# bhmm/bhmm

Hardware: NVIDIA B200
Metric: Baum-Welch EM throughput (frames x iterations per second) (higher is better)
Workload: dtype f64

## Files before the change

bhmm_b200/csrc/engine.cu:

```cuda
#include <algorithm>
#include <cstdio>
#include <cstdlib>
#include <cstring>

#include "host_common.h"
#include "../../include/bhmm_b200.h"

struct bhmm_b200_batch {
    int K = 0, N = 0;
    long long rows = 0;
    std::vector<long long> offsets;
    int chunk = 0, warm_f = 0, warm_b = 0, warm_min = 32;
    int req_chunk = 0, req_warm = 0;
    int vit_phase = 0;
    bool vit_map_chunked = false;
    std::vector<int> vit_end;
    bool lane = false;
    bool no_alpha = false;
    double* d_g0buf = nullptr;
    int partial_rows = 0;
    HostPlan plan, segplan;
    Arena arena;
    bool carved = false;
    char* cw_base = nullptr;
// ... 65 lines not shown
        b->d_sigma = (double*)(base + o_sg);
        b->d_partials = (double*)(base + o_part);
        b->d_g0buf = (double*)(base + o_g0);
        b->d_err = (int*)(base + o_err);
        b->d_alpha = (double*)(base + o_alpha);
        b->d_F = (unsigned char*)(base + o_F);
        b->d_vflag = (unsigned*)(base + o_vflag);
        b->cw_base = base + o_cw;
    }
    return cv.off + 256;
}

int batch_carve(bhmm_b200_batch* b, cudaStream_t st)
{
    if (b->carved) return BHMM_OK;
    const size_t need = batch_layout(b, nullptr);
    RC_TRY(b->arena.ensure(need));
    batch_layout(b, b->arena.base);
    RC_TRY(chainwork_setup(b->w, b->plan, b->N, b->warm_f, b->cw_base, st));
    const int ns = b->segplan.n;
    CUDA_TRY(cudaMemcpyAsync(b->d_offsets, b->offsets.data(), sizeof(long long) * (b->K + 1), cudaMemcpyHostToDevice, st));
    CUDA_TRY(cudaMemcpyAsync((void*)b->seg.row0, b->segplan.row0.data(), sizeof(long long) * ns, cudaMemcpyHostToDevice, st));
    CUDA_TRY(cudaMemcpyAsync((void*)b->seg.len, b->segplan.len.data(), sizeof(int) * ns, cudaMemcpyHostToDevice, st));
    CUDA_TRY(cudaMemcpyAsync((void*)b->seg.t0, b->segplan.t0.data(), sizeof(int) * ns, cudaMemcpyHostToDevice, st));
    CUDA_TRY(cudaMemcpyAsync((void*)b->seg.T, b->segplan.T.data(), sizeof(int) * ns, cudaMemcpyHostToDevice, st));
    CUDA_TRY(cudaStreamSynchronize(st));
    b->carved = true;
    return BHMM_OK;
}

void batch_plan(bhmm_b200_batch* b, int chunk, int warm)
{
    b->req_chunk = chunk;
    b->req_warm = warm;
    const int w = warm > 0 ? warm : (b->lane ? auto_warm_lane(b->N) : auto_warm(b->N));
    b->chunk = chunk > 0 ? chunk : (b->lane ? auto_chunk_lane(b->rows, b->N, w) : auto_chunk(b->rows, b->N, w));
    if (chunk <= 0) {
        int sms = 148, dev = 0;
        if (cudaGetDevice(&dev) == cudaSuccess) cudaDeviceGetAttribute(&sms, cudaDevAttrMultiProcessorCount, dev);
        int tthreads = 32, tcpb = 1;
        team_shape(b->N, &tthreads, &tcpb);
        const long long cap = b->lane ? (long long)sms * lane_blocks_per_sm(b->N, EM_GAUSS) * lane_threads()
                                      : (long long)backward_stats_grid(b->N, 1 << 28) * tcpb;
        auto count = [&](long long c) {
            long long n = 0;
            for (int k = 0; k < b->K; ++k) {
                const long long own = b->own_lo.empty() ? b->offsets[k + 1] - b->offsets[k] : b->own_hi[k] - b->own_lo[k];
                n += (own + c - 1) / c;
            }
            return n;
        };
        if (b->lane) {
            for (int it = 0; it < 200; ++it) {
                if (count(b->chunk) <= cap || b->chunk >= (1 << 30)) break;
                b->chunk = (int)std::min<long long>((long long)b->chunk + std::max(1, b->chunk / 100), 1 << 30);
            }
        } else {
            long long maxT = 1;
            for (int k = 0; k < b->K; ++k) maxT = std::max(maxT, b->offsets[k + 1] - b->offsets[k]);
            const long long lo_c = std::max<long long>(64, 2LL * w);
            double best_cost = 1e300;
            long long best_c = std::max<long long>(maxT, 1);
            for (int m = 1; m <= 32; ++m) {
                if (count(maxT) > (long long)m * cap) continue;
                long long lo = std::min(lo_c, maxT), hi = maxT;
                while (lo < hi) {
                    const long long mid = (lo + hi) / 2;
                    if (count(mid) <= (long long)m * cap) hi = mid; else lo = mid + 1;
                }
                const double cost = (double)m * ((double)lo + (lo < maxT ? (double)w : 0.0));
                if (cost < best_cost * 0.98) { best_cost = cost; best_c = lo; }
            }
            b->chunk = (int)std::min<long long>(best_c, 1 << 30);
        }
    }
    b->warm_f = b->warm_b = w;
    b->warm_min = warm > 0 ? warm : 32;
    build_plan(b->offsets.data(), b->K, b->chunk, b->plan, b->own_lo.empty() ? nullptr : b->own_lo.data(),
               b->own_hi.empty() ? nullptr : b->own_hi.data());
    build_plan(b->offsets.data(), b->K, SEG_FRAMES, b->segplan);
    b->carved = false;
}

int upload_small(double* dst, const double* src, size_t n, cudaStream_t st)
{
    CUDA_TRY(cudaMemcpyAsync(dst, src, sizeof(double) * n, cudaMemcpyHostToDevice, st));
    return BHMM_OK;
}

struct ScanGuard {
    bhmm_b200_batch* b;
    ScanGuard(bhmm_b200_batch* b_, const Emission& em, int emkind) : b(b_)
    {
        const int N = b->N;
        static int off = -1;
        if (off < 0) { const char* e = getenv("BHMM_B200_EXACT_SCAN"); off = (e && e[0] == '0') ? 1 : 0; }
        if (off || !exact_scan_ok(N) || !b->w.chunked) return;
        b->w.scan = [this, &em, emkind, N](int dir, cudaStream_t st) -> int {
            const size_t need = exact_scan_bytes(b->w.n_total, N);
            if (b->scan.ensure(need) != BHMM_OK) { bhmm_set_error(BHMM_ERR_NO_MEM, "exact scan: device memory for the chain operators"); return BHMM_ERR_NO_MEM; }
            Chains all = b->w.ch;
            return launch_exact_scan(all, b->w.n_total, em, emkind, b->d_A, N, dir, dir > 0 ? b->w.he_f : b->w.he_b,
                                     reinterpret_cast<double*>(b->scan.base), st);
        };
    }
    ~ScanGuard() { b->w.scan = nullptr; }
};

struct RepairTolGuard {
    ChainWork& w;
    explicit RepairTolGuard(ChainWork& w_) : w(w_) { w.repair_tol = g_repair_tol; }
    ~RepairTolGuard() { w.repair_tol = 0.0; }
};

void begin_info(bhmm_b200_batch* b)
{
    b->info = RunInfo();
    b->info.chains = b->plan.n;
    b->info.chunk = b->chunk;
    b->info.warm = b->warm_f;
}

int prepare_discrete(bhmm_b200_batch* b, const double* B, int M, Emission& em, cudaStream_t st)
{
    const int N = b->N;
    RC_TRY(b->disc.ensure(sizeof(double) * 2 * (size_t)N * M + 512));
    double* stage = (double*)b->disc.base;
    double* Bt = stage + (((size_t)N * M + 31) & ~(size_t)31);
    CUDA_TRY(cudaMemcpyAsync(stage, B, sizeof(double) * (size_t)N * M, cudaMemcpyHostToDevice, st));
    RC_TRY(launch_transpose(stage, N, M, Bt, st));
    LAUNCHED(1);
    em.Bt = Bt;
    em.M = M;
    return BHMM_OK;
}

int estep_common(bhmm_b200_batch* b, Emission& em, int emkind, const double* A, const double* pi, const double* mu,
                 const double* sigma, double* d_gamma, double* d_stats, double* d_Bnum, cudaStream_t st)
{
    const int N = b->N;
    if (b->no_alpha) { bhmm_set_error(BHMM_ERR_UNSUPPORTED, "Viterbi-only batch: no forward variables"); return BHMM_ERR_UNSUPPORTED; }
    RC_TRY(upload_small(b->d_A, A, (size_t)N * N, st));
    RC_TRY(upload_small(b->d_pi, pi, N, st));
    b->w.ch.warm = b->warm_f;
    ScanGuard scan_guard(b, em, emkind);
    RepairTolGuard repair_guard(b->w);
    LaneArgs la{};
    LaneHostParams hp{A, pi, mu, sigma};
    if (b->lane) {
        la.obs = em.obs; la.sym = em.sym; la.Bt = em.Bt; la.M = em.M; la.ignore_outliers = em.ignore_outliers;
        la.alpha_il = b->d_alpha; la.Lmax = b->chunk; la.alpha_rm = nullptr;
        la.chain_ll = b->w.chain_ll; la.g0buf = b->d_g0buf; la.partials = b->d_partials;
        la.Bnum = d_Bnum; la.gamma = d_gamma;
    }
    static int optimistic = -1;
    if (optimistic < 0) { const char* e = getenv("BHMM_B200_OPTIMISTIC"); optimistic = (e && e[0] == '1') ? 1 : 0; }
    auto launch_fwd = [&](const Chains& ch, cudaStream_t s2) -> int {
        if (b->lane) {
            LaneArgs x = la;
            x.ch = ch; x.hand_used = b->w.hu_f; x.hand_end = b->w.he_f;
            return launch_lane(x, hp, N, emkind, LANE_FORWARD, s2);
        }
        FwdArgs a{};
        a.ch = ch; a.em = em; a.N = N; a.A = b->d_A; a.pi = b->d_pi; a.alpha = b->d_alpha;
        a.chain_ll = b->w.chain_ll; a.hand_used = b->w.hu_f; a.hand_end = b->w.he_f;
        return launch_forward_team(a, emkind, s2);
    };
    auto launch_bwd = [&](const Chains& ch, cudaStream_t s2) -> int {
        if (b->lane) {
            LaneArgs x = la;
            x.ch = ch; x.hand_used = b->w.hu_b; x.hand_end = b->w.he_b;
            return launch_lane(x, hp, N, emkind, LANE_BACKWARD_STATS, s2);
        }
        BwdArgs a{};
        a.ch = ch;
        a.em = em; a.N = N; a.grid = b->stats_grid; a.A = b->d_A;
        a.alpha = b->d_alpha; a.gamma = d_gamma; a.Bnum = d_Bnum; a.partials = b->d_partials;
        a.hand_used = b->w.hu_b; a.hand_end = b->w.he_b;
        return launch_backward_team(a, emkind, true, s2);
    };
    auto finalize = [&]() -> int {
        const int prow = b->lane ? lane_blocks(b->w.n_total) : b->stats_grid;
        RC_TRY(launch_finalize_stats(b->d_partials, prow, b->w.chain_ll, b->w.n_total, b->d_A, N, d_stats, st));
        LAUNCHED(1);
        if (b->lane) {
            RC_TRY(launch_add_gamma0(b->w.ch, b->w.n_total, N, b->d_g0buf, d_stats, st));
            LAUNCHED(1);
        }
        return BHMM_OK;
    };
    if (optimistic && b->w.chunked) {
        Chains all = b->w.ch;
        all.list = nullptr; all.n = b->w.n_total; all.exact = 0; all.warmv = nullptr;
        b->w.need_f = b->w.need_b = 0.0;
        if (b->profile) cudaEventRecord(b->ev[0], st);
        all.warm = b->warm_f;
        RC_TRY(launch_fwd(all, st));
        LAUNCHED(1);
        RC_TRY(certify_async(b->w, N, +1, st));
        if (b->profile) { cudaEventRecord(b->ev[1], st); cudaEventRecord(b->ev[2], st); }
        if (d_Bnum) CUDA_TRY(cudaMemsetAsync(d_Bnum, 0, sizeof(double) * (size_t)N * em.M, st));
        all.warm = b->warm_b;
        RC_TRY(launch_bwd(all, st));
        LAUNCHED(1);
        if (b->profile) cudaEventRecord(b->ev[3], st);
        RC_TRY(certify_async(b->w, N, -1, st));
        RC_TRY(finalize());
        CUDA_TRY(cudaStreamSynchronize(st));
        double wf = 0.0, wb = 0.0;
        const long long ff = certify_collect(b->w, +1, &wf), fb = certify_collect(b->w, -1, &wb);
        if (ff == 0 && fb == 0) {
            b->info.worst_f = wf; b->info.worst_b = wb;
            b->warm_f = adapt_warm(b->warm_f, b->w.need_f, wf, false, b->warm_min, b->plan.maxT, b->edge_f);
            b->warm_b = adapt_warm(b->warm_b, b->w.need_b, wb, false, b->warm_min, b->plan.maxT, b->edge_b);
            b->info.warm = std::max(b->warm_f, b->warm_b);
            return BHMM_OK;
        }
        b->info.rerun += (double)b->w.n_total;
        b->w.ch.warm = b->warm_f;
    }

    if (b->profile) cudaEventRecord(b->ev[0], st);
    RC_TRY(run_chains_certified(b->w, N, +1, launch_fwd, b->info, st));
    if (b->profile) cudaEventRecord(b->ev[1], st);
    if (b->w.chunked) b->warm_f = adapt_warm(b->warm_f, b->w.need_f, b->info.worst_f, b->info.fix_f > 0, b->warm_min, b->plan.maxT, b->edge_f);

    b->w.need_b = 0.0;
    bool exact_bwd = false;
    for (int attempt = 0;; ++attempt) {
        Chains all = b->w.ch;
        all.list = nullptr; all.n = b->w.n_total; all.exact = exact_bwd ? 1 : 0; all.warm = b->warm_b; all.warmv = nullptr;
        if (d_Bnum) CUDA_TRY(cudaMemsetAsync(d_Bnum, 0, sizeof(double) * (size_t)N * em.M, st));
        if (b->profile) cudaEventRecord(b->ev[2], st);
        RC_TRY(launch_bwd(all, st));
        LAUNCHED(1);
        if (b->profile) cudaEventRecord(b->ev[3], st);
        if (!b->w.chunked) break;
        const long long nfail = certify_sync(b->w, N, -1, &b->info.worst_b, st, exact_bwd ? EXACT_SCAN_TOL : 0.0);
        if (nfail < 0) { bhmm_set_error(BHMM_ERR_CUDA, cudaGetErrorString(cudaGetLastError())); return BHMM_ERR_CUDA; }
        if (nfail == 0) { b->warm_b = adapt_warm(b->warm_b, b->w.need_b, b->info.worst_b, false, b->warm_min, b->plan.maxT, b->edge_b); break; }
        if (exact_bwd || b->warm_b >= b->plan.maxT) {
            char msg[160];
            snprintf(msg, sizeof(msg), "backward hand-overs not certified (%lld chains, worst mismatch %.3g%s)", nfail, b->info.worst_b,
                     exact_bwd ? ", after the exact scan" : "");
            bhmm_set_error(BHMM_ERR_NOT_CERTIFIED, msg);
            return BHMM_ERR_NOT_CERTIFIED;
        }
        b->info.fix_b += 1;
        b->info.rerun += (double)b->w.n_total;
        if (attempt >= 1 && b->w.scan) {
            RC_TRY(b->w.scan(-1, st));
            LAUNCHED(2);
            b->w.scans += 1;
            exact_bwd = true;
            continue;
        }
        b->warm_b = adapt_warm(b->warm_b, b->w.need_b, b->info.worst_b, true, b->warm_min, b->plan.maxT, b->edge_b);
    }
    RC_TRY(finalize());
    b->info.warm = std::max(b->warm_f, b->warm_b);
    return BHMM_OK;
}

int finish_stream(cudaStream_t st)
{
    cudaError_t e = cudaStreamSynchronize(st);
    if (e == cudaSuccess) e = cudaGetLastError();
    if (e != cudaSuccess) { bhmm_set_error(BHMM_ERR_CUDA, cudaGetErrorString(e)); return BHMM_ERR_CUDA; }
    return BHMM_OK;
}

void collect_times(bhmm_b200_batch* b)
{
    if (!b->profile) return;
    float f = 0.f, g = 0.f, t = 0.f;
    cudaEventElapsedTime(&f, b->ev[0], b->ev[1]);
    cudaEventElapsedTime(&g, b->ev[2], b->ev[3]);
    cudaEventElapsedTime(&t, b->ev[0], b->ev[3]);
    b->kernel_ms[0] = f; b->kernel_ms[1] = g; b->kernel_ms[2] = t;
}

int gibbs_common(bhmm_b200_batch* b, Emission& em, int emkind, const double* A, const double* pi, const double* mu,
                 const double* sigma, const double* d_u,
                 unsigned long long seed, unsigned long long sweep, int* d_path, long long* d_counts, double* d_sums,
                 double* loglik_host, cudaStream_t st)
{
    const int N = b->N;
    if (!b->own_lo.empty()) { bhmm_set_error(BHMM_ERR_UNSUPPORTED, "hidden-path sampling needs whole trajectories (batch has owned ranges)"); return BHMM_ERR_UNSUPPORTED; }
    if (b->no_alpha) { bhmm_set_error(BHMM_ERR_UNSUPPORTED, "Viterbi-only batch: no forward variables"); return BHMM_ERR_UNSUPPORTED; }
    if (N > 256) { bhmm_set_error(BHMM_ERR_UNSUPPORTED, "sampling supports N <= 256"); return BHMM_ERR_UNSUPPORTED; }
    RC_TRY(upload_small(b->d_A, A, (size_t)N * N, st));
    RC_TRY(upload_small(b->d_pi, pi, N, st));
    b->w.ch.warm = b->warm_f;
    ScanGuard scan_guard(b, em, emkind);
    if (b->lane) {
        LaneArgs la{};
        LaneHostParams hp{A, pi, mu, sigma};
        la.obs = em.obs; la.sym = em.sym; la.Bt = em.Bt; la.M = em.M; la.ignore_outliers = em.ignore_outliers;
        la.alpha_il = b->d_alpha; la.Lmax = b->chunk; la.chain_ll = b->w.chain_ll;
        la.hand_used = b->w.hu_f; la.hand_end = b->w.he_f;
        RC_TRY(run_chains_certified(b->w, N, +1, [&](const Chains& ch, cudaStream_t s2) {
            LaneArgs x = la;
            x.ch = ch;
            return launch_lane(x, hp, N, emkind, LANE_FORWARD, s2);
        }, b->info, st));
        if (b->w.chunked) b->warm_f = adapt_warm(b->warm_f, b->w.need_f, b->info.worst_f, b->info.fix_f > 0, b->warm_min, b->plan.maxT, b->edge_f);
// ... 408 lines not shown
```

bhmm_b200/csrc/kernels.h:

```cpp
#pragma once
#include "common.cuh"

struct FwdArgs {
    Chains ch;
    Emission em;
    int N;
    int cpb;
    const double* A;
    const double* pi;
    double* alpha;
    double* chain_ll;
    double* hand_used;
    double* hand_end;
};

struct BwdArgs {
    Chains ch;
    Emission em;
    int N;
    int cpb;
    int grid;
    const double* A;
    double* beta;
    const double* alpha;
    double* gamma;
    double* Bnum;
    double* partials;
    double* hand_used;
    double* hand_end;
};

struct VitArgs {
    Emission em;
    int N;
    int cpb;
    int K;
    const long long* offsets;
    const double* A;
    const double* pi;
    void* backptr;
    int* path;
};

struct VitChainArgs {
    Chains ch;
    Emission em;
    int N;
    const double* A;
    const double* pi;
    void* backptr;
    double* hand_used;
    double* hand_end;
    unsigned* flagmap;
    double margin_min;
};

constexpr int LANE_MAX_N = 16;
template <int N>
struct LaneParams {
    double A[N * N];
    double pi[N];
    double mu[N];
    double isg[N];
    double nrm[N];
    double nrml[N];
};
struct LaneHostParams {
    const double* A;
    const double* pi;
    const double* mu;
    const double* sigma;
};
struct LaneArgs {
    Chains ch;
    const double* obs;
    const int* sym;
    const double* Bt;
    int M;
    int ignore_outliers;
    double* alpha_il;
    int Lmax;
    double* alpha_rm;
    double* chain_ll;
    double* hand_used;
    double* hand_end;
    double* g0buf;
    double* partials;
    double* Bnum;
    double* gamma;
    const double* u_row;
    unsigned long long seed, sweep;
    int* path;
    unsigned char* smap;
    const int* enter;
    int* coal;
    long long* counts;
    int* err;
};
enum { LANE_FORWARD = 0, LANE_FORWARD_ROWMAJOR = 1, LANE_BACKWARD_STATS = 2, LANE_SAMPLE_MAP = 3, LANE_SAMPLE_FIX = 4,
       LANE_QUERY_BLOCKS = 5 };
int lane_blocks_per_sm(int N, int em);
int lane_threads();
int launch_lane_sum_moments(const double* partials, int rows, int N, double* sums, cudaStream_t st);
bool lane_supported(int N, int em);
int lane_blocks(int n_chains);
int launch_lane(const LaneArgs& a, const LaneHostParams& hp, int N, int em, int what, cudaStream_t st);
int launch_add_gamma0(const Chains& ch, int n_total, int N, const double* g0buf, double* stats, cudaStream_t st);

void team_shape(int N, int* threads, int* cpb);
int launch_forward_team(const FwdArgs& a, int em, cudaStream_t st);
int launch_backward_team(const BwdArgs& a, int em, bool stats, cudaStream_t st);
int backward_stats_grid(int N, int n_chains);
int launch_viterbi_team(const VitArgs& a, int em, cudaStream_t st);

bool panel_enabled(int N);
void panel_shape(int N, int* threads, int* chains_per_row);
int panel_stats_rows(int N, int n_chains);
bool panel_forward_ok(const FwdArgs& a, int em);
bool panel_backward_ok(const BwdArgs& a, int em);
int launch_forward_panel(const FwdArgs& a, int em, cudaStream_t st);
int launch_backward_stats_panel(const BwdArgs& a, int em, cudaStream_t st);
bool panel_viterbi_ok(int N);
int launch_viterbi_panel(const VitArgs& a, int em, cudaStream_t st);
bool exact_scan_ok(int N);
size_t exact_scan_bytes(int n_chains, int N);
int launch_exact_scan(const Chains& all, int n_total, const Emission& em, int emkind, const double* dA, int N, int dir,
                      double* he, double* ops, cudaStream_t st);
bool lane_viterbi_ok(int N);
int launch_viterbi_chain_lane(const VitChainArgs& a, int em, cudaStream_t st);
bool panel_viterbi_chain_ok(int N);
int launch_viterbi_chain(const VitChainArgs& a, int em, cudaStream_t st);
int launch_viterbi_path_flags(const unsigned* flagmap, const int* path, const long long* offsets, int K, long long rows,
                              int* counter, cudaStream_t st);

int launch_gaussian_pobs(const double* obs, const double* mu, const double* sigma, int N, long long rows,
                         int ignore_outliers, double* pobs, cudaStream_t st);
int launch_discrete_pobs(const int* sym, const double* Bt, int N, int M, long long rows, int ignore_outliers,
                         double* pobs, cudaStream_t st);
int launch_state_probabilities(const double* alpha, const double* beta, int N, long long rows, double* gamma,
                               cudaStream_t st);
int launch_state_counts(const double* gamma, int N, long long rows, double* counts, double* scratch, int* blocks,
                        cudaStream_t st);
int state_counts_blocks(long long rows);
int launch_transition_counts(const double* alpha, const double* beta, const double* A, const double* pobs, int N,
                             int T, double* C, double* scratch, cudaStream_t st);
int transition_counts_blocks(int T);
int launch_update_pout(const int* sym, const double* w, long long rows, int N, int M, double* pout, cudaStream_t st);
int launch_mstep_hmm(const double* stats, const double* mu_old, int N, int gauss, double mincount, double* out, cudaStream_t st);
int launch_mstep_rows(const double* Bnum, int N, int M, double* B, double* Bt, cudaStream_t st);
int launch_transpose(const double* in, int R, int Cc, double* out, cudaStream_t st);

int launch_certify(const Chains& ch, int n_total, int N, int dir, const double* hand_used, const double* hand_end,
                   double tol, double tol_fail, int* fail_list, unsigned long long* out, cudaStream_t st);
int launch_finalize_stats(const double* partials, int grid, const double* chain_ll, int n_chains, const double* A,
                          int N, double* stats, cudaStream_t st);

int launch_sample_table(const double* alpha, const double* A, const double* u, const long long* offsets, int K,
                        int N, long long rows, unsigned char* F, int* err, cudaStream_t st);
int launch_sample_table_philox(const double* alpha, const double* A, unsigned long long seed, unsigned long long ctr,
                               const long long* offsets, int K, int N, long long rows, unsigned char* F, int* err,
                               cudaStream_t st);
int launch_chase(const unsigned char* F, const Chains& seg, int N, unsigned char* seg_map, int* seg_enter, int* path,
                 cudaStream_t st);
int launch_chase_link(const Chains& seg, int N, const unsigned char* seg_map, int* seg_enter, cudaStream_t st);
int launch_path_stats(const int* path, const double* obs, const long long* offsets, int K, int N, long long rows,
                      long long* Cint, long long* n0, long long* cnt, double* so, double* soo, cudaStream_t st);
int launch_symbol_histogram(const int* path, const int* sym, long long rows, int N, int M, long long* hist,
                            cudaStream_t st);
```

bhmm_b200/csrc/lane_kernels.cuh:

```cuda
#pragma once
#include "common.cuh"
#include "kernels.h"

namespace {

constexpr int LANE_THREADS = 64;
constexpr unsigned FULL = 0xffffffffu;

#ifndef LANE_MINB_F
#define LANE_MINB_F 4
#endif
#ifndef LANE_MINB_B
#define LANE_MINB_B 4
#endif
#ifndef LANE_FOLD_NRM
#define LANE_FOLD_NRM 1
#endif
#ifndef LANE_CONST_SMEM
#define LANE_CONST_SMEM 1
#endif
#ifndef LANE_KEEP_F
#define LANE_KEEP_F 40
#endif
#ifndef LANE_EXP_TABLE
// ... 112 lines not shown
        for (int j = 0; j < N; ++j) {
            const int ni = __double2loint(t[j]);
            p[j] = __longlong_as_double(__double_as_longlong(p[j]) + ((long long)ni << 52));
#if !LANE_FOLD_NRM
            p[j] *= P.nrml[j];
#endif
        }
    } else {
#pragma unroll
        for (int j = 0; j < N; ++j) t[j] = fma(x[j], EXPK2[4], MAGIC);
#pragma unroll
        for (int j = 0; j < N; ++j) r[j] = fma(t[j] - MAGIC, -EXPK2[5], x[j]);
        double tb[N];
#pragma unroll
        for (int j = 0; j < N; ++j) {
            const int kk = __double2loint(t[j]);
            const double e = LANE_EXP_REPL ? P.tab[((kk & 31) << 4) + (threadIdx.x & 15)] : P.tab[kk & 31];
            tb[j] = __hiloint2double(__double2hiint(e) + (kk << 15), __double2loint(e));
        }
#pragma unroll
        for (int j = 0; j < N; ++j) p[j] = fma(EXPK2[0], r[j], EXPK2[1]);
#pragma unroll
        for (int k = 2; k < 4; ++k) {
#pragma unroll
            for (int j = 0; j < N; ++j) p[j] = fma(p[j], r[j], EXPK2[k]);
        }
#pragma unroll
        for (int j = 0; j < N; ++j) p[j] = fma(p[j], r[j], 1.0);
#pragma unroll
        for (int j = 0; j < N; ++j) p[j] = fma(p[j], r[j], 1.0);
#pragma unroll
        for (int j = 0; j < N; ++j) {
            p[j] *= tb[j];
#if !LANE_FOLD_NRM
            p[j] *= P.nrml[j];
#endif
        }
    }
    {
        unsigned umax = (unsigned)__double2hiint(x[0]);
        int smax = __double2hiint(x[0]);
#pragma unroll
        for (int j = 1; j < N; ++j) {
            umax = max(umax, (unsigned)__double2hiint(x[j]));
            smax = max(smax, __double2hiint(x[j]));
        }
        if (umax > 0xC0862000u || smax > 0x40862000) {
#pragma unroll
            for (int j = 0; j < N; ++j) {
                const unsigned hx = (unsigned)__double2hiint(x[j]);
#if LANE_FOLD_NRM
                if (x[j] - P.nrm[j] < -745.1332191019412) {
                    p[j] = 0.0;
                } else
#endif
                if (hx >= 0xC0875000u && hx <= 0xFFF00000u) {
                    p[j] = 0.0;
                } else if ((hx & 0x7fffffffu) > 0x40862000u) {
                    p[j] = slow_exp(x[j]);
#if !LANE_FOLD_NRM
                    p[j] *= P.nrml[j];
#endif
                }
            }
        }
    }
    int nzbits = 0;
#pragma unroll
    for (int j = 0; j < N; ++j) nzbits |= __double2hiint(p[j]) | __double2loint(p[j]);
    const bool anynz = (nzbits & 0x7fffffff) != 0 || nzbits != 0;
    if (ignore_outliers && !anynz) {
#pragma unroll
        for (int j = 0; j < N; ++j) p[j] = 1.0;
    }
}

template <int N>
__device__ __forceinline__ void emission_disc(const LaneArgs& a, int sym, double (&p)[N])
{
    const double* src = a.Bt + (long long)sym * N;
    bool anynz = false;
#pragma unroll
    for (int j = 0; j < N; ++j) { p[j] = __ldg(src + j); anynz |= (p[j] != 0.0); }
    if (a.ignore_outliers && !anynz) {
#pragma unroll
        for (int j = 0; j < N; ++j) p[j] = 1.0;
    }
}

struct LogAcc {
    double prod = 1.0;
    long long esum = 0;
    double slow = 0.0;
    __device__ __forceinline__ void add(double c)
    {
        const int ec = (int)((__double_as_longlong(c) >> 52) & 0x7ff);
        if (ec == 0 || ec == 0x7ff || c < 0.0) { slow += log(c); return; }
        prod *= c;
        const long long b = __double_as_longlong(prod);
        esum += (long long)((b >> 52) & 0x7ff) - 1023;
        prod = __longlong_as_double((b & 0x800fffffffffffffLL) | 0x3ff0000000000000LL);
    }
    __device__ __forceinline__ double value() const { return (double)esum * 0.693147180559945309417 + log(prod) + slow; }
};

#ifndef LANE_LAZY
#define LANE_LAZY 480
#endif
template <int N>
__device__ __forceinline__ int top_exponent(const double (&v)[N])
{
    int h[N];
#pragma unroll
    for (int j = 0; j < N; ++j) h[j] = __double2hiint(v[j]);
#pragma unroll
    for (int w = 1; w < N; w *= 3) {
#pragma unroll
        for (int j = 0; j < N; j += 3 * w) {
            if (j + w < N) h[j] = max(h[j], h[j + w]);
            if (j + 2 * w < N) h[j] = max(h[j], h[j + 2 * w]);
        }
    }
    return h[0] >> 20;
}
__device__ __forceinline__ bool regular_exponent(int e) { return e >= 64 && e < 2040; }
template <int N>
__device__ __forceinline__ int rescale_pow2(double (&v)[N], int e)
{
    if ((unsigned)(e - 1023) <= (unsigned)LANE_LAZY) return 0;
    const int shift = max(e - (1023 + LANE_LAZY / 2), -1022);
    const double f = __hiloint2double((1023 - shift) << 20, 0);
#pragma unroll
    for (int j = 0; j < N; ++j) v[j] *= f;
    return shift;
}

__device__ __forceinline__ long long il_base(int c, int Lmax, int NP2)
{
    return ((long long)(c >> 5) * Lmax * NP2 << 5) + (c & 31);
}

template <int V> struct BoolTag2 { static constexpr int value = V; };

template <int N>
struct ConstView {
    const double* A;
    const double* pi;
    const double* mu;
    const double* isg;
    const double* nrm;
    const double* nrml;
    const double* tab;
    const double* At;
};
template <int N>
constexpr int lane_const_doubles() { return (int)(sizeof(LaneParams<N>) / sizeof(double)) + 32 * kExpCopies + (LANE_AT_B ? N * N : 0); }
template <int N>
__device__ __forceinline__ ConstView<N> make_const_view(const LaneParams<N>& P, double* smem)
{
    constexpr int TOT = sizeof(LaneParams<N>) / sizeof(double);
    const double* src = reinterpret_cast<const double*>(&P);
    for (int k = threadIdx.x; k < TOT; k += blockDim.x) smem[k] = src[k];
    for (int k = threadIdx.x; k < 32 * kExpCopies; k += blockDim.x) {
        const int j = k / kExpCopies;
        const double e = EXPT[j];
        smem[TOT + k] = __hiloint2double(__double2hiint(e) - (j << 15), __double2loint(e));
    }
    if (LANE_AT_B) {
        for (int k = threadIdx.x; k < N * N; k += blockDim.x) smem[TOT + 32 * kExpCopies + k] = src[(k % N) * N + k / N];
    }
    __syncthreads();
    ConstView<N> v;
    v.tab = smem + TOT;
    v.At = smem + TOT + 32 * kExpCopies;

#if LANE_CONST_SMEM == 2
    v.A = P.A;
#else
    v.A = smem;
#endif
    v.pi = smem + N * N; v.mu = v.pi + N; v.isg = v.mu + N; v.nrm = v.isg + N; v.nrml = v.nrm + N;
    return v;
}
enum { PATH_GENERAL = 0, PATH_CHAIN = 1, PATH_WARM = 2 };

template <int N, int EM, bool ROWMAJOR>
__global__ void __launch_bounds__(LANE_THREADS, LANE_MINB_F)
k_forward_lane(const __grid_constant__ LaneParams<N> Pk, const LaneArgs a)
{
    constexpr int NP2 = (N + 1) / 2;
    constexpr int PF = LANE_PF;
#if LANE_CONST_SMEM
    __shared__ double cs[lane_const_doubles<N>()];
    const ConstView<N> P = make_const_view<N>(Pk, cs);
#else
    const LaneParams<N>& P = Pk;
#endif
    const int idx = blockIdx.x * blockDim.x + threadIdx.x;
    const bool have = idx < a.ch.n;
    int c = 0, len = 0, t0 = 0, tstart = 0, mode = 0;
    long long trow = 0;
    if (have) {
        c = a.ch.list ? a.ch.list[idx] : idx;
        len = a.ch.len[c];
        t0 = a.ch.t0[c];
        trow = a.ch.row0[c] - t0;
        if (t0 == 0) { tstart = 0; mode = 0; }
        else if (a.ch.exact) { tstart = t0 - 1; mode = 2; }
        else { tstart = max(0, t0 - (a.ch.warmv ? a.ch.warmv[c] : a.ch.warm)); mode = (tstart == 0) ? 0 : 1; }
    }
    const int maxpre = __reduce_max_sync(FULL, have ? (t0 - tstart) : 0);
    const int total = maxpre + __reduce_max_sync(FULL, len);
    const int tend = t0 + len;

    double al[N];
#pragma unroll
    for (int j = 0; j < N; ++j) al[j] = 0.0;
    if (have && mode == 2) {
#pragma unroll
        for (int j = 0; j < N; ++j) al[j] = a.hand_end[(long long)(c - 1) * N + j];
    }
    long long esum = 0;
    double slow = 0.0, log_start = 0.0, log_end = 0.0;
    double2* il = reinterpret_cast<double2*>(a.alpha_il) + il_base(c, a.Lmax, NP2);

    auto fetch = [&](int s) -> double {
        int t = t0 - maxpre + s;
        if (!have) return 0.0;
        t = min(max(t, tstart), tend - 1);
#ifdef LANE_DEBUG_NOFETCH
        return 0.37 + 1e-3 * (t & 1023);
#endif
#if LANE_OBS_PREFETCH
        if (EM == EM_GAUSS) prefetch_l1(a.obs + trow + min(t + 16, tend - 1));
        else prefetch_l1(a.sym + trow + min(t + 32, tend - 1));
#endif
        if (EM == EM_GAUSS) return __ldg(a.obs + trow + t);
        return __longlong_as_double((long long)__ldg(a.sym + trow + t));
    };
    double ring[PF];
#pragma unroll
    for (int k = 0; k < PF; ++k) ring[k] = fetch(k);
    auto emission = [&](double rawv, double (&pv)[N]) {
        if (EM == EM_GAUSS) emission_gauss<N, LANE_EXP_TABLE>(P, rawv, a.ignore_outliers, pv);
        else emission_disc<N>(a, (int)__double_as_longlong(rawv), pv);
    };

    constexpr int KEEP = (LANE_KEEP_F < N * N) ? LANE_KEEP_F : N * N;
    double Areg[KEEP > 0 ? KEEP : 1];
#pragma unroll
    for (int k = 0; k < KEEP; ++k) Areg[k] = P.A[k];
    auto Aat = [&](int k) -> double { return (k < KEEP) ? Areg[k] : P.A[k]; };

    auto propagate = [&](double (&v)[N], const double (&p)[N]) {
#pragma unroll
        for (int j = 0; j < N; ++j) v[j] = al[0] * Aat(j);
#pragma unroll
        for (int i = 1; i < N; ++i) {
#pragma unroll
            for (int j = 0; j < N; ++j) v[j] = fma(al[i], Aat(i * N + j), v[j]);
        }
#pragma unroll
        for (int j = 0; j < N; ++j) v[j] *= p[j];
    };

    auto step = [&](auto path_tag, int t, double raw, bool on) {
        constexpr int PATH = decltype(path_tag)::value;
        if (!on) return;
        double p[N];
        const bool init = (PATH == PATH_GENERAL) && (t == tstart);
        double v[N];
        if (init && mode == 2) {
#pragma unroll
            for (int j = 0; j < N; ++j) v[j] = al[j];
        } else {
            emission(raw, p);
            if (init) {
#pragma unroll
                for (int j = 0; j < N; ++j) v[j] = (mode == 0) ? P.pi[j] * p[j] : p[j];
            } else {
                propagate(v, p);
            }
        }
        const bool inchain = (PATH == PATH_CHAIN) || (PATH == PATH_GENERAL && t >= t0);
        const int e = top_exponent<N>(v);
        if (regular_exponent(e)) {
            const int shift = rescale_pow2<N>(v, e);
#pragma unroll
            for (int j = 0; j < N; ++j) al[j] = v[j];
            if (inchain) esum += shift;
        } else {
            const double csum = tree_sum<N>(v);
            const double rc = (csum != 0.0) ? 1.0 / csum : 1.0;
#pragma unroll
            for (int j = 0; j < N; ++j) al[j] = v[j] * rc;
            if (inchain) slow += log(csum);
        }
        if (inchain) {
            if (ROWMAJOR) {
                double* dst = a.alpha_rm + (trow + t) * N;
#pragma unroll
                for (int j = 0; j < N; ++j) dst[j] = al[j];
            } else {
                double2* dst = il + ((long long)(t - t0) * NP2 << 5);
#ifdef LANE_DEBUG_NOSTORE
                if (al[0] == 1.2345e-200)
#endif
#pragma unroll
                for (int jp = 0; jp < NP2; ++jp)
                    __stcs(dst + (jp << 5), make_double2(al[2 * jp], (2 * jp + 1 < N) ? al[2 * jp + 1] : 0.0));
            }
        }
        if (PATH == PATH_GENERAL) {
            if (t == tend - 1 || t == t0 - 1) {
                const double sig = tree_sum<N>(al);
                const double rs = (sig != 0.0) ? 1.0 / sig : 1.0;
                double* dst = (t == tend - 1) ? a.hand_end : a.hand_used;
                if (t == tend - 1) log_end = log(sig);
                else log_start = (sig != 0.0) ? log(sig) : 0.0;
#pragma unroll
                for (int j = 0; j < N; ++j) dst[(long long)c * N + j] = al[j] * rs;
            }
        }
    };

    auto next_raw = [&](int s) -> double {
        const double raw = ring[0];
#pragma unroll
        for (int k = 0; k + 1 < PF; ++k) ring[k] = ring[k + 1];
        ring[PF - 1] = fetch(s + PF);
        return raw;
    };
    int s = 0;
    while (s < total) {
        const int t = t0 - maxpre + s;
        const bool on = have && t >= tstart && t < tend;
        const int cls = !on ? 0 : ((t == tstart || t == tend - 1 || t == t0 - 1) ? 3 : (t >= t0 ? 1 : 2));
        const unsigned m1 = __ballot_sync(FULL, cls == 1), m2 = __ballot_sync(FULL, cls == 2),
                       m3 = __ballot_sync(FULL, cls == 3);
        if (m3 || (m1 && m2) || !(m1 | m2)) {
            step(BoolTag2<PATH_GENERAL>(), t, next_raw(s), on);
            ++s;
            continue;
        }
        const int rem = (cls == 1) ? tend - 2 - t : (cls == 2) ? t0 - 2 - t : (have && t < tstart) ? tstart - 1 - t : 0x7fffffff;
        const int run = 1 + __reduce_min_sync(FULL, rem);
        if (m1) {
#pragma unroll kUnrollF
            for (int k = 0; k < run; ++k, ++s) step(BoolTag2<PATH_CHAIN>(), t0 - maxpre + s, next_raw(s), on);
        } else {
            for (int k = 0; k < run; ++k, ++s) step(BoolTag2<PATH_WARM>(), t0 - maxpre + s, next_raw(s), on);
        }
    }
    if (have) a.chain_ll[c] = (log_end - log_start) + (double)esum * 0.693147180559945309417 + slow;
}

template <int N, int G, int NH>
__device__ __forceinline__ double pick_row(const double (&arr)[N], int qsel, int ii)
{
    double v = arr[ii];
#pragma unroll
    for (int qq = 1; qq < G; ++qq)
        if (qq * NH + ii < N) v = (qsel == qq) ? arr[qq * NH + ii] : v;
    return v;
}

template <int N, int EM, int G>
__global__ void __launch_bounds__(LANE_THREADS, LANE_MINB_B)
k_backward_stats_lane(const __grid_constant__ LaneParams<N> Pk, const LaneArgs a)
{
    constexpr int NP2 = (N + 1) / 2;
    constexpr int NH = (N + G - 1) / G;
    constexpr int PF = LANE_PF;
    constexpr int NSTAT = N * N + 4 * N;
    __shared__ double red[(LANE_THREADS / 32) * NSTAT];
#if LANE_CONST_SMEM
    __shared__ double cs[lane_const_doubles<N>()];
    const ConstView<N> P = make_const_view<N>(Pk, cs);
#else
    const LaneParams<N>& P = Pk;
#endif

    const int idx = blockIdx.x * blockDim.x + threadIdx.x;
    const int lane = threadIdx.x & 31;
    const int q = lane & (G - 1);
    const bool have = idx < a.ch.n;
    int c = 0, len = 0, t0 = 0, T = 0, e = 0, fs = 0, mode = 0;
    long long trow = 0;
    if (have) {
        c = a.ch.list ? a.ch.list[idx] : idx;
        len = a.ch.len[c];
        t0 = a.ch.t0[c];
        T = a.ch.T[c];
        trow = a.ch.row0[c] - t0;
        e = t0 + len;
        if (e >= T) fs = T - 1;
        else if (a.ch.exact) { fs = e; mode = 2; }
        else fs = min(T - 1, e + (a.ch.warmv ? a.ch.warmv[c] : a.ch.warm) - 1);
    }
    const int maxpre = __reduce_max_sync(FULL, have ? (fs - (e - 1)) : 0);
    const int total = maxpre + __reduce_max_sync(FULL, len);

    double Cq[NH][N];
    double sg[NH], sgd[NH], sgdd[NH], muq[NH];
#pragma unroll
    for (int ii = 0; ii < NH; ++ii) {
        sg[ii] = sgd[ii] = sgdd[ii] = 0.0;
        muq[ii] = P.mu[min(q * NH + ii, N - 1)];
#pragma unroll
        for (int j = 0; j < N; ++j) Cq[ii][j] = 0.0;
    }
    double bt[N];
#pragma unroll
    for (int j = 0; j < N; ++j) bt[j] = 0.0;
    const double2* il = reinterpret_cast<const double2*>(a.alpha_il) + il_base(c, a.Lmax, NP2);

    auto frame_of = [&](int s) -> int { return (e - 1) + maxpre - s; };
    auto fetch = [&](int s) -> double {
        int f = frame_of(s);
        if (!have) return 0.0;
        f = min(max(f, t0), T - 1);
#if LANE_OBS_PREFETCH
        if (EM == EM_GAUSS) prefetch_l1(a.obs + trow + max(f - 16, t0));
        else prefetch_l1(a.sym + trow + max(f - 32, t0));
#endif
        if (EM == EM_GAUSS) return __ldg(a.obs + trow + f);
        return __longlong_as_double((long long)__ldg(a.sym + trow + f));
    };
    double ring[PF];
#pragma unroll
    for (int k = 0; k < PF; ++k) ring[k] = fetch(k);
    auto emission = [&](double rawv, double (&pv)[N]) {
        if (EM == EM_GAUSS) emission_gauss<N, LANE_EXP_TABLE>(P, rawv, a.ignore_outliers, pv);
        else emission_disc<N>(a, (int)__double_as_longlong(rawv), pv);
    };
    double raw_next = 0.0;

    constexpr bool XCH = (G >= LANE_XCH_MIN_G);
    constexpr int XU = NH;
    __shared__ double2 xch[XCH ? (LANE_THREADS / 32) * G * XU * 32 : 1];
    double2* const xw = xch + (threadIdx.x >> 5) * (G * XU * 32);
    auto accumulate = [&](const double (&w)[N], const double (&u)[N], const double (&gam)[N], double o_f) {
        if (XCH) {
#pragma unroll
            for (int blk = 0; blk < G; ++blk) {
                double L[2 * NH];
#pragma unroll
                for (int ii = 0; ii < NH; ++ii) {
                    L[ii] = (blk * NH + ii < N) ? u[(blk * NH + ii < N) ? blk * NH + ii : 0] : 0.0;
                    L[NH + ii] = (blk * NH + ii < N) ? gam[(blk * NH + ii < N) ? blk * NH + ii : 0] : 0.0;
                }
#pragma unroll
                for (int k = 0; k < XU; ++k) xw[(blk * XU + k) * 32 + lane] = make_double2(L[2 * k], L[2 * k + 1]);
            }
            __syncwarp();
        }
#pragma unroll
        for (int d = 0; d < G; ++d) {
            double ur[NH], gr[NH];
            double od;
            if (XCH) {
                double L[2 * NH];
#pragma unroll
                for (int k = 0; k < XU; ++k) {
                    const double2 v = xw[(q * XU + k) * 32 + (lane ^ d)];
                    L[2 * k] = v.x;
                    L[2 * k + 1] = v.y;
                }
#pragma unroll
                for (int ii = 0; ii < NH; ++ii) { ur[ii] = L[ii]; gr[ii] = L[NH + ii]; }
                od = (d == 0) ? o_f : __shfl_xor_sync(FULL, o_f, d);
            } else if (d == 0) {
#pragma unroll
                for (int ii = 0; ii < NH; ++ii) {
                    ur[ii] = pick_row<N, G, NH>(u, q, ii);
                    gr[ii] = pick_row<N, G, NH>(gam, q, ii);
                }
                od = o_f;
            } else {
#pragma unroll
                for (int ii = 0; ii < NH; ++ii) {
                    ur[ii] = __shfl_xor_sync(FULL, pick_row<N, G, NH>(u, q ^ d, ii), d);
                    gr[ii] = __shfl_xor_sync(FULL, pick_row<N, G, NH>(gam, q ^ d, ii), d);
                }
                od = __shfl_xor_sync(FULL, o_f, d);
            }
#pragma unroll
            for (int j = 0; j < N; ++j) {
                const double wj = (d == 0) ? w[j] : __shfl_xor_sync(FULL, w[j], d);
#pragma unroll
                for (int ii = 0; ii < NH; ++ii) Cq[ii][j] = fma(ur[ii], wj, Cq[ii][j]);
            }
#pragma unroll
            for (int ii = 0; ii < NH; ++ii) {
                sg[ii] += gr[ii];
                if (EM == EM_GAUSS) {
                    const double dd = od - muq[ii];
                    sgd[ii] = fma(gr[ii], dd, sgd[ii]);
                    sgdd[ii] = fma(gr[ii], dd * dd, sgdd[ii]);
                }
            }
        }
        if (XCH) __syncwarp();
    };

    auto back_propagate = [&](double (&b)[N], double (&w)[N], const double (&p)[N]) {
#pragma unroll
        for (int j = 0; j < N; ++j) w[j] = p[j] * bt[j];
#pragma unroll
        for (int i = 0; i < N; ++i) b[i] = (LANE_AT_B ? P.At[i] : P.A[i * N]) * w[0];
#pragma unroll
        for (int j = 1; j < N; ++j) {
#pragma unroll
            for (int i = 0; i < N; ++i) b[i] = fma(LANE_AT_B ? P.At[j * N + i] : P.A[i * N + j], w[j], b[i]);
        }
    };

    auto step = [&](auto path_tag, int f, double raw, bool on) {
        constexpr int PATH = decltype(path_tag)::value;
        const bool act = (PATH == PATH_CHAIN) || on;
        const bool init = (PATH == PATH_GENERAL) && on && f == fs;
        const bool emit = (PATH == PATH_CHAIN) || (PATH == PATH_GENERAL && on && f < e);
        double w[N], u[N], gam[N];
        double o_f = 0.0;
        double p[N];
        if (PATH == PATH_GENERAL) {
#pragma unroll
            for (int j = 0; j < N; ++j) { w[j] = 0.0; u[j] = 0.0; gam[j] = 0.0; }
        }
        if (act) {
            double2 a2[NP2];
            if (emit) {
                const double2* src = il + ((long long)(on ? f - t0 : 0) * NP2 << 5);
#pragma unroll
                for (int jp = 0; jp < NP2; ++jp) a2[jp] = __ldcs(src + (jp << 5));
#if LANE_ALPHA_PREFETCH
                if (N <= LANE_ALPHA_PREFETCH_MAXN && on && f > t0) {
#pragma unroll
                    for (int jp = 0; jp < NP2; ++jp) prefetch_l1(src - (NP2 << 5) + (jp << 5));
                }
#endif
            }
            double b[N];
            if (init) {
                if (mode == 2) {
#pragma unroll
                    for (int j = 0; j < N; ++j) b[j] = a.hand_end[(long long)(c + 1) * N + j];
                } else {
#pragma unroll
                    for (int j = 0; j < N; ++j) b[j] = 1.0;
                }
            } else {
                emission(raw_next, p);
                back_propagate(b, w, p);
            }
            const int eb = top_exponent<N>(b);
            if (emit) {
                double al[N], gi[N];
#pragma unroll
                for (int jp = 0; jp < NP2; ++jp) {
                    al[2 * jp] = a2[jp].x;
                    if (2 * jp + 1 < N) al[2 * jp + 1] = a2[jp].y;
                }
#pragma unroll
                for (int i = 0; i < N; ++i) gi[i] = al[i] * b[i];
                const double S = tree_sum<N>(gi);
                const double rS = (PATH == PATH_CHAIN && !on) ? 0.0 : 1.0 / S;
#pragma unroll
                for (int i = 0; i < N; ++i) {
                    u[i] = al[i] * rS;
                    gam[i] = gi[i] * rS;
                }
                if (EM == EM_GAUSS) o_f = raw;
                if (PATH == PATH_GENERAL && f == 0) {
#pragma unroll
                    for (int i = 0; i < N; ++i) a.g0buf[(long long)c * N + i] = gam[i];
                }
                if (a.gamma && on) {
                    double* dst = a.gamma + (trow + f) * N;
#pragma unroll
                    for (int i = 0; i < N; ++i) dst[i] = gam[i];
                }
                if (EM == EM_DISC && a.Bnum && on) {
                    const int sy = (int)__double_as_longlong(raw);
#pragma unroll
                    for (int i = 0; i < N; ++i) atomicAdd(a.Bnum + (long long)i * a.M + sy, gam[i]);
                }
            }
            if (regular_exponent(eb)) {
                rescale_pow2<N>(b, eb);
#pragma unroll
                for (int i = 0; i < N; ++i) bt[i] = b[i];
            } else {
                const double sb = tree_sum<N>(b);
                const double rsb = (sb != 0.0) ? 1.0 / sb : 1.0;
#pragma unroll
                for (int i = 0; i < N; ++i) bt[i] = b[i] * rsb;
            }
            if (PATH == PATH_GENERAL && (f == e || (f == t0 && t0 > 0))) {
                const double sb = tree_sum<N>(bt);
                const double rsb = (sb != 0.0) ? 1.0 / sb : 1.0;
                double* dst = (f == e) ? a.hand_used : a.hand_end;
#pragma unroll
                for (int i = 0; i < N; ++i) dst[(long long)c * N + i] = bt[i] * rsb;
            }
            raw_next = raw;
        }
        if (PATH != PATH_WARM) accumulate(w, u, gam, o_f);
    };

    auto next_raw = [&](int s) -> double {
        const double raw = ring[0];
#pragma unroll
        for (int k = 0; k + 1 < PF; ++k) ring[k] = ring[k + 1];
        ring[PF - 1] = fetch(s + PF);
        return raw;
    };
    int s = 0;
    while (s < total) {
        const int f = frame_of(s);
        const bool on = have && f <= fs && f >= t0;
        const int cls = !on ? 0 : ((f == fs || f == e || f == t0 || f == 0) ? 3 : (f < e ? 1 : 2));
        const unsigned m1 = __ballot_sync(FULL, cls == 1), m2 = __ballot_sync(FULL, cls == 2),
                       m3 = __ballot_sync(FULL, cls == 3);
        if (m3 || (m1 && m2) || !(m1 | m2)) {
            step(BoolTag2<PATH_GENERAL>(), f, next_raw(s), on);
            ++s;
            continue;
        }
        const int rem = (cls == 1) ? f - t0 - 1 : (cls == 2) ? f - e - 1 : (have && f > fs) ? f - fs - 1 : 0x7fffffff;
        const int run = 1 + __reduce_min_sync(FULL, rem);
        if (m1) {
#pragma unroll kUnrollB
            for (int k = 0; k < run; ++k, ++s) step(BoolTag2<PATH_CHAIN>(), frame_of(s), next_raw(s), on);
        } else {
            for (int k = 0; k < run; ++k, ++s) step(BoolTag2<PATH_WARM>(), frame_of(s), next_raw(s), on);
        }
    }

#pragma unroll
    for (int off = G; off < 32; off <<= 1) {
#pragma unroll
        for (int ii = 0; ii < NH; ++ii) {
            sg[ii] += __shfl_xor_sync(FULL, sg[ii], off);
            sgd[ii] += __shfl_xor_sync(FULL, sgd[ii], off);
            sgdd[ii] += __shfl_xor_sync(FULL, sgdd[ii], off);
#pragma unroll
            for (int j = 0; j < N; ++j) Cq[ii][j] += __shfl_xor_sync(FULL, Cq[ii][j], off);
        }
    }
    double* myred = red + (threadIdx.x >> 5) * NSTAT;
    if (lane < G) {
#pragma unroll
        for (int ii = 0; ii < NH; ++ii) {
            const int i = q * NH + ii;
            if (i < N) {
#pragma unroll
                for (int j = 0; j < N; ++j) myred[i * N + j] = Cq[ii][j];
                myred[N * N + i] = 0.0;
                myred[N * N + N + i] = sg[ii];
                myred[N * N + 2 * N + i] = sgd[ii];
                myred[N * N + 3 * N + i] = sgdd[ii];
            }
        }
    }
    __syncthreads();
    double* out = a.partials + (long long)blockIdx.x * NSTAT;
    for (int k = threadIdx.x; k < NSTAT; k += blockDim.x) {
        double v = 0.0;
#pragma unroll
        for (int wp = 0; wp < LANE_THREADS / 32; ++wp) v += red[wp * NSTAT + k];
        out[k] = v;
    }
}

__device__ __forceinline__ void lane_philox_round(uint32_t& c0, uint32_t& c1, uint32_t& c2, uint32_t& c3, uint32_t k0,
                                                  uint32_t k1)
{
    const uint32_t hi0 = __umulhi(0xD2511F53u, c0), lo0 = 0xD2511F53u * c0;
    const uint32_t hi1 = __umulhi(0xCD9E8D57u, c2), lo1 = 0xCD9E8D57u * c2;
    const uint32_t n0 = hi1 ^ c1 ^ k0, n1 = lo1, n2 = hi0 ^ c3 ^ k1, n3 = lo0;
    c0 = n0; c1 = n1; c2 = n2; c3 = n3;
}

__device__ __forceinline__ double lane_philox_uniform(unsigned long long seed, unsigned long long ctr, long long row)
{
    uint32_t c0 = (uint32_t)row, c1 = (uint32_t)((unsigned long long)row >> 32);
    uint32_t c2 = (uint32_t)ctr, c3 = (uint32_t)(ctr >> 32);
    uint32_t k0 = (uint32_t)seed, k1 = (uint32_t)(seed >> 32);
#pragma unroll
    for (int r = 0; r < 10; ++r) {
        lane_philox_round(c0, c1, c2, c3, k0, k1);
        k0 += 0x9E3779B9u;
        k1 += 0xBB67AE85u;
    }
    const unsigned long long bits = ((unsigned long long)c0 << 32) | c1;
    return (double)(bits >> 11) * (1.0 / 9007199254740992.0);
}

template <int N, bool EXACT>
__device__ __forceinline__ int lane_draw(const double (&al)[N], const double* __restrict__ A_s, int v, double r,
                                         bool last, bool& bad)
{
    double pv[N];
#pragma unroll
    for (int i = 0; i < N; ++i) pv[i] = last ? al[i] : __dmul_rn(al[i], A_s[i * N + v]);
    if (EXACT) {
        double s = 0.0;
#pragma unroll
        for (int i = 0; i < N; ++i) s = __dadd_rn(s, pv[i]);
        double acc = 0.0;
        int pick = -1;
#pragma unroll
        for (int i = 0; i < N; ++i) {
            acc = __dadd_rn(acc, __ddiv_rn(pv[i], s));
            if (pick < 0 && acc >= r) pick = i;
        }
        if (pick < 0) { pick = N - 1; bad = true; }
        return pick;
    }
    double s = pv[0];
#pragma unroll
    for (int i = 1; i < N; ++i) s += pv[i];
    const double thr = r * s;
    double acc = 0.0;
    int cnt = 0;
#pragma unroll
    for (int i = 0; i < N; ++i) {
        acc += pv[i];
        cnt += (acc < thr) ? 1 : 0;
    }
    if (!(s > 0.0)) bad = true;
    return min(cnt, N - 1);
}

template <int N, int EM, bool EXACT, bool FIXPASS>
__global__ void __launch_bounds__(LANE_THREADS)
k_sample_lane(const __grid_constant__ LaneParams<N> Pk, const LaneArgs a)
{
    constexpr int NP2 = (N + 1) / 2;
    constexpr int NI = N * N + 2 * N;
    extern __shared__ unsigned char smraw[];
    double* A_s = reinterpret_cast<double*>(smraw);
    double* mom = A_s + N * N;
    int* cnts = reinterpret_cast<int*>(mom + 2 * N * LANE_THREADS);
    for (int k = threadIdx.x; k < N * N; k += blockDim.x) A_s[k] = Pk.A[k];
    for (int k = threadIdx.x; k < 2 * N * LANE_THREADS; k += blockDim.x) mom[k] = 0.0;
    for (int k = threadIdx.x; k < NI * LANE_THREADS; k += blockDim.x) cnts[k] = 0;
    __syncthreads();

    const int tid = threadIdx.x;
    const int idx = blockIdx.x * blockDim.x + tid;
    const bool have = idx < a.ch.n;
    int c = 0, len = 0, t0 = 0, T = 0, e = 0;
    long long trow = 0;
    if (have) {
        c = idx;
        len = a.ch.len[c];
        t0 = a.ch.t0[c];
        T = a.ch.T[c];
        trow = a.ch.row0[c] - t0;
        e = t0 + len;
    }
    const double2* il = reinterpret_cast<const double2*>(a.alpha_il) + il_base(c, a.Lmax, NP2);
    bool bad = false;

    auto load_alpha = [&](int f, double (&al)[N]) {
        const double2* src = il + ((long long)(f - t0) * NP2 << 5);
#pragma unroll
        for (int jp = 0; jp < NP2; ++jp) {
            const double2 v2 = __ldcs(src + (jp << 5));
            al[2 * jp] = v2.x;
            if (2 * jp + 1 < N) al[2 * jp + 1] = v2.y;
        }
    };
    auto prefetch_step = [&](int f) {
        const int fa = f - LANE_SAMPLE_AHEAD;
        if (fa >= t0) {
            const double2* src = il + ((long long)(fa - t0) * NP2 << 5);
#pragma unroll
            for (int jp = 0; jp < NP2; ++jp) prefetch_l1(src + (jp << 5));
        }
        const int fo = max(f - 16, t0);
        if (EM == EM_GAUSS) prefetch_l1(a.obs + trow + fo);
        if (a.u_row) prefetch_l1(a.u_row + trow + fo);
    };
    auto uniform = [&](int f) -> double {
        return a.u_row ? __ldg(a.u_row + trow + f) : lane_philox_uniform(a.seed, a.sweep, trow + f);
    };
// ... 172 lines not shown
```

Before: 12.33 billion.

## Run early warm-up steps of lane forward/backward passes in FP32

Adds an FP32 path for the first part of the warm-up region in the lane forward and backward kernels. It uses float copies of A, mu, scaled inverse sigma and norm constants stored in shared memory, ex2.approx for Gaussian emissions, and exponent-based renormalization. The goal is to cut FP64 arithmetic in warm-up frames, whose values only seed the chain state and are then refined in FP64. The path is on by default and can be disabled with an environment variable. It risks small accuracy changes in the warm start and uses slightly more shared memory.

```diff
diff --git a/bhmm_b200/csrc/engine.cu b/bhmm_b200/csrc/engine.cu
--- a/bhmm_b200/csrc/engine.cu
+++ b/bhmm_b200/csrc/engine.cu
@@ -241,6 +241,9 @@
         la.alpha_il = b->d_alpha; la.Lmax = b->chunk; la.alpha_rm = nullptr;
         la.chain_ll = b->w.chain_ll; la.g0buf = b->d_g0buf; la.partials = b->d_partials;
         la.Bnum = d_Bnum; la.gamma = d_gamma;
+        static int warm_fp32 = -1;
+        if (warm_fp32 < 0) { const char* e = getenv("BHMM_B200_WARM_FP32"); warm_fp32 = (e && e[0] == '0') ? 0 : 1; }
+        la.warm_fp32 = b->own_lo.empty() ? warm_fp32 : 0;
     }
     static int optimistic = -1;
     if (optimistic < 0) { const char* e = getenv("BHMM_B200_OPTIMISTIC"); optimistic = (e && e[0] == '1') ? 1 : 0; }
diff --git a/bhmm_b200/csrc/kernels.h b/bhmm_b200/csrc/kernels.h
--- a/bhmm_b200/csrc/kernels.h
+++ b/bhmm_b200/csrc/kernels.h
@@ -88,6 +88,7 @@
     double* partials;
     double* Bnum;
     double* gamma;
+    int warm_fp32;
     const double* u_row;
     unsigned long long seed, sweep;
     int* path;
diff --git a/bhmm_b200/csrc/lane_kernels.cuh b/bhmm_b200/csrc/lane_kernels.cuh
--- a/bhmm_b200/csrc/lane_kernels.cuh
+++ b/bhmm_b200/csrc/lane_kernels.cuh
@@ -288,9 +288,15 @@
     const double* nrml;
     const double* tab;
     const double* At;
+    const float* A32;
+    const float* mu32;
+    const float* isg32;
+    const float* nrm32;
 };
 template <int N>
-constexpr int lane_const_doubles() { return (int)(sizeof(LaneParams<N>) / sizeof(double)) + 32 * kExpCopies + (LANE_AT_B ? N * N : 0); }
+constexpr int lane_const_doubles_fp64() { return (int)(sizeof(LaneParams<N>) / sizeof(double)) + 32 * kExpCopies + (LANE_AT_B ? N * N : 0); }
+template <int N>
+constexpr int lane_const_doubles() { return lane_const_doubles_fp64<N>() + (N * N + 3 * N + 1) / 2; }
 template <int N>
 __device__ __forceinline__ ConstView<N> make_const_view(const LaneParams<N>& P, double* smem)
 {
@@ -305,10 +311,20 @@
     if (LANE_AT_B) {
         for (int k = threadIdx.x; k < N * N; k += blockDim.x) smem[TOT + 32 * kExpCopies + k] = src[(k % N) * N + k / N];
     }
+    float* f32 = reinterpret_cast<float*>(smem + lane_const_doubles_fp64<N>());
+    for (int k = threadIdx.x; k < N * N + 3 * N; k += blockDim.x) {
+        double x;
+        if (k < N * N) x = P.A[k];
+        else if (k < N * N + N) x = P.mu[k - N * N];
+        else if (k < N * N + 2 * N) x = P.isg[k - N * N - N] * 1.2011224087864498;
+        else x = P.nrm[k - N * N - 2 * N] * 1.4426950408889634;
+        f32[k] = (float)x;
+    }
     __syncthreads();
     ConstView<N> v;
     v.tab = smem + TOT;
     v.At = smem + TOT + 32 * kExpCopies;
+    v.A32 = f32; v.mu32 = f32 + N * N; v.isg32 = v.mu32 + N; v.nrm32 = v.isg32 + N;
 
 #if LANE_CONST_SMEM == 2
     v.A = P.A;
@@ -319,6 +335,54 @@
     return v;
 }
 enum { PATH_GENERAL = 0, PATH_CHAIN = 1, PATH_WARM = 2 };
+
+constexpr int kWarm32Div = 4;
+__device__ __forceinline__ float ex2_approx(float x)
+{
+    float y;
+    asm("ex2.approx.ftz.f32 %0, %1;" : "=f"(y) : "f"(x));
+    return y;
+}
+template <int N>
+__device__ __forceinline__ void warm32_renorm(float (&v)[N])
+{
+    int h = __float_as_int(v[0]);
+#pragma unroll
+    for (int j = 1; j < N; ++j) h = max(h, __float_as_int(v[j]));
+    const int e = h >> 23;
+    if ((unsigned)(e - (127 - 60)) > 120u) {
+        const bool bad = e <= 0 || e >= 254;
+        const float f = bad ? 0.0f : __int_as_float((254 - e) << 23);
+#pragma unroll
+        for (int j = 0; j < N; ++j) v[j] = bad ? 1.0f : v[j] * f;
+    }
+}
+template <int N>
+__device__ __forceinline__ void warm32_from_double(const double (&d)[N], float (&v)[N])
+{
+    const int e = top_exponent<N>(d);
+    const bool bad = e <= 0 || e >= 2046;
+    const double f = bad ? 0.0 : __hiloint2double((2046 - e) << 20, 0);
+#pragma unroll
+    for (int j = 0; j < N; ++j) v[j] = bad ? 1.0f : __double2float_rn(d[j] * f);
+}
+template <int N, int EM, typename CV>
+__device__ __forceinline__ void warm32_emission(const CV& P, const LaneArgs& a, double raw, float (&p)[N])
+{
+    if (EM == EM_GAUSS) {
+        const float o = __double2float_rn(raw);
+#pragma unroll
+        for (int j = 0; j < N; ++j) {
+            const float d = (o - P.mu32[j]) * P.isg32[j];
+            p[j] = ex2_approx(fmaf(-d, d, P.nrm32[j]));
+        }
+    } else {
+        double pd[N];
+        emission_disc<N>(a, (int)__double_as_longlong(raw), pd);
+#pragma unroll
+        for (int j = 0; j < N; ++j) p[j] = __double2float_rn(pd[j]);
+    }
+}
 
 template <int N, int EM, bool ROWMAJOR>
 __global__ void __launch_bounds__(LANE_THREADS, LANE_MINB_F)
@@ -348,6 +412,7 @@
     const int maxpre = __reduce_max_sync(FULL, have ? (t0 - tstart) : 0);
     const int total = maxpre + __reduce_max_sync(FULL, len);
     const int tend = t0 + len;
+    const int w32end = (LANE_CONST_SMEM && a.warm_fp32 && have && mode == 1) ? tstart + 1 + (t0 - tstart) / kWarm32Div : tstart;
 
     double al[N];
 #pragma unroll
@@ -471,21 +536,45 @@
     while (s < total) {
         const int t = t0 - maxpre + s;
         const bool on = have && t >= tstart && t < tend;
-        const int cls = !on ? 0 : ((t == tstart || t == tend - 1 || t == t0 - 1) ? 3 : (t >= t0 ? 1 : 2));
+        const int cls = !on ? 0 : ((t == tstart || t == tend - 1 || t == t0 - 1) ? 3 : (t >= t0 ? 1 : (t < w32end ? 4 : 2)));
         const unsigned m1 = __ballot_sync(FULL, cls == 1), m2 = __ballot_sync(FULL, cls == 2),
-                       m3 = __ballot_sync(FULL, cls == 3);
-        if (m3 || (m1 && m2) || !(m1 | m2)) {
+                       m3 = __ballot_sync(FULL, cls == 3), m4 = __ballot_sync(FULL, cls == 4);
+        if (m3 || (m1 != 0) + (m2 != 0) + (m4 != 0) != 1) {
             step(BoolTag2<PATH_GENERAL>(), t, next_raw(s), on);
             ++s;
             continue;
         }
-        const int rem = (cls == 1) ? tend - 2 - t : (cls == 2) ? t0 - 2 - t : (have && t < tstart) ? tstart - 1 - t : 0x7fffffff;
+        const int rem = (cls == 1) ? tend - 2 - t : (cls == 2) ? t0 - 2 - t : (cls == 4) ? w32end - 1 - t
+                      : (have && t < tstart) ? tstart - 1 - t : 0x7fffffff;
         const int run = 1 + __reduce_min_sync(FULL, rem);
         if (m1) {
 #pragma unroll kUnrollF
             for (int k = 0; k < run; ++k, ++s) step(BoolTag2<PATH_CHAIN>(), t0 - maxpre + s, next_raw(s), on);
+        } else if (m2) {
+            for (int k = 0; k < run; ++k, ++s) step(BoolTag2<PATH_WARM>(), t0 - maxpre + s, next_raw(s), on);
         } else {
-            for (int k = 0; k < run; ++k, ++s) step(BoolTag2<PATH_WARM>(), t0 - maxpre + s, next_raw(s), on);
+#if LANE_CONST_SMEM
+            float v32[N];
+            warm32_from_double<N>(al, v32);
+            for (int k = 0; k < run; ++k, ++s) {
+                float p[N], v[N];
+                warm32_emission<N, EM>(P, a, next_raw(s), p);
+#pragma unroll
+                for (int j = 0; j < N; ++j) v[j] = v32[0] * P.A32[j];
+#pragma unroll
+                for (int i = 1; i < N; ++i) {
+#pragma unroll
+                    for (int j = 0; j < N; ++j) v[j] = fmaf(v32[i], P.A32[i * N + j], v[j]);
+                }
+#pragma unroll
+                for (int j = 0; j < N; ++j) v32[j] = v[j] * p[j];
+                warm32_renorm<N>(v32);
+            }
+            if (on) {
+#pragma unroll
+                for (int j = 0; j < N; ++j) al[j] = (double)v32[j];
+            }
+#endif
         }
     }
     if (have) a.chain_ll[c] = (log_end - log_start) + (double)esum * 0.693147180559945309417 + slow;
@@ -536,6 +625,7 @@
     }
     const int maxpre = __reduce_max_sync(FULL, have ? (fs - (e - 1)) : 0);
     const int total = maxpre + __reduce_max_sync(FULL, len);
+    const int lo32 = (LANE_CONST_SMEM && a.warm_fp32 && have && mode == 0 && fs < T - 1) ? fs - (fs - e) / kWarm32Div : fs + 1;
 
     double Cq[NH][N];
     double sg[NH], sgd[NH], sgdd[NH], muq[NH];
@@ -756,21 +846,51 @@
     while (s < total) {
         const int f = frame_of(s);
         const bool on = have && f <= fs && f >= t0;
-        const int cls = !on ? 0 : ((f == fs || f == e || f == t0 || f == 0) ? 3 : (f < e ? 1 : 2));
+        const int cls = !on ? 0 : ((f == fs || f == e || f == t0 || f == 0) ? 3 : (f < e ? 1 : (f >= lo32 ? 4 : 2)));
         const unsigned m1 = __ballot_sync(FULL, cls == 1), m2 = __ballot_sync(FULL, cls == 2),
-                       m3 = __ballot_sync(FULL, cls == 3);
-        if (m3 || (m1 && m2) || !(m1 | m2)) {
+                       m3 = __ballot_sync(FULL, cls == 3), m4 = __ballot_sync(FULL, cls == 4);
+        if (m3 || (m1 != 0) + (m2 != 0) + (m4 != 0) != 1) {
             step(BoolTag2<PATH_GENERAL>(), f, next_raw(s), on);
             ++s;
             continue;
         }
-        const int rem = (cls == 1) ? f - t0 - 1 : (cls == 2) ? f - e - 1 : (have && f > fs) ? f - fs - 1 : 0x7fffffff;
+        const int rem = (cls == 1) ? f - t0 - 1 : (cls == 2) ? f - e - 1 : (cls == 4) ? f - lo32
+                      : (have && f > fs) ? f - fs - 1 : 0x7fffffff;
         const int run = 1 + __reduce_min_sync(FULL, rem);
         if (m1) {
 #pragma unroll kUnrollB
             for (int k = 0; k < run; ++k, ++s) step(BoolTag2<PATH_CHAIN>(), frame_of(s), next_raw(s), on);
+        } else if (m2) {
+            for (int k = 0; k < run; ++k, ++s) step(BoolTag2<PATH_WARM>(), frame_of(s), next_raw(s), on);
         } else {
-            for (int k = 0; k < run; ++k, ++s) step(BoolTag2<PATH_WARM>(), frame_of(s), next_raw(s), on);
+#if LANE_CONST_SMEM
+            float b32[N];
+            warm32_from_double<N>(bt, b32);
+            double rn = raw_next;
+            for (int k = 0; k < run; ++k, ++s) {
+                const double raw = next_raw(s);
+                float p[N], w[N], b[N];
+                warm32_emission<N, EM>(P, a, rn, p);
+#pragma unroll
+                for (int j = 0; j < N; ++j) w[j] = p[j] * b32[j];
+#pragma unroll
+                for (int i = 0; i < N; ++i) b[i] = P.A32[i * N] * w[0];
+#pragma unroll
+                for (int j = 1; j < N; ++j) {
+#pragma unroll
+                    for (int i = 0; i < N; ++i) b[i] = fmaf(P.A32[i * N + j], w[j], b[i]);
+                }
+#pragma unroll
+                for (int i = 0; i < N; ++i) b32[i] = b[i];
+                warm32_renorm<N>(b32);
+                rn = raw;
+            }
+            if (on) {
+                raw_next = rn;
+#pragma unroll
+                for (int i = 0; i < N; ++i) bt[i] = (double)b32[i];
+            }
+#endif
         }
     }
 
```

New measurement: 12.55 billion, median of 6. +1.7%, better.
